# JakubValtar/basisu_rs

Measured on AMD Instinct MI355X. Metric: M 4x4 blocks/s UASTC->BC7 4096x4096, higher is better.
Workload: dtype u8

## Files before the change

### basisu_rs_amd/csrc/bu_capi_slice.hpp

```cpp
#pragma once
extern "C" {

size_t bu_target_block_bytes(bu_target target)
{
    switch (target) {
    case BU_TARGET_ASTC:
    case BU_TARGET_BC7:
    case BU_TARGET_ETC2:
    case BU_TARGET_BC5_RG:
    case BU_TARGET_EAC_RG11:
    case BU_TARGET_BC3_RGBA: return 16;
    case BU_TARGET_ETC1:
    case BU_TARGET_BC4_R:
    case BU_TARGET_EAC_R11:
    case BU_TARGET_BC1_RGB: return 8;
    case BU_TARGET_RGBA32: return 64;
    default: return 0;
    }
}

const char* bu_status_string(bu_status st)
{
    switch (st) {
    case BU_OK: return "ok";
// ... 132 lines not shown
    if (st != BU_ERR_INVALID_MODE && st != BU_ERR_INVALID_PATTERN && st != BU_ERR_INDEX_RANGE && st != BU_ERR_UNSUPPORTED) return BU_ERR_ARGUMENT;
    if (first_bad_block) *first_bad_block = word >> 8;
    return static_cast<bu_status>(st);
}

bu_status bu_host_alloc(bu_context* ctx, size_t bytes, void** out_ptr)
{
    if (!ctx || !out_ptr) return BU_ERR_ARGUMENT;
    *out_ptr = nullptr;
    if (bytes == 0) return BU_OK;
    BU_HIP(ctx, hipSetDevice(ctx->device));
    BU_HIP(ctx, hipHostMalloc(out_ptr, bytes, hipHostMallocDefault));
    return BU_OK;
}

bu_status bu_host_free(bu_context* ctx, void* ptr)
{
    if (!ctx) return BU_ERR_ARGUMENT;
    if (!ptr) return BU_OK;
    BU_HIP(ctx, hipSetDevice(ctx->device));
    BU_HIP(ctx, hipHostFree(ptr));
    return BU_OK;
}

bu_status bu_uastc_transcode_device(bu_context* ctx, bu_target target, const void* d_in, size_t n_blocks, void* d_out,
                                    size_t blocks_per_row, uint64_t block_index_base, uint64_t* d_status, void* stream)
{
    if (!ctx || (n_blocks && (!d_in || !d_out))) return BU_ERR_ARGUMENT;
    if (bu_target_block_bytes(target) == 0) return BU_ERR_ARGUMENT;
    if (target == BU_TARGET_RGBA32 && blocks_per_row == 0) return BU_ERR_ARGUMENT;
    if (target == BU_TARGET_RGBA32 && n_blocks % blocks_per_row != 0) return BU_ERR_ARGUMENT;
    return bu_launch_uastc(ctx, target, d_in, n_blocks, d_out, blocks_per_row, block_index_base, d_status, static_cast<hipStream_t>(stream), 0, -1);
}

}
namespace {
bu_status bu_batch_runs(bu_context* ctx, bu_target target, size_t n_slices, const void* const* d_in, const size_t* n_blocks, void* const* d_out,
                        size_t blocks_per_row, const uint64_t* index_base, std::vector<BuRun>& runs)
{
    if (!ctx || (n_slices && (!d_in || !n_blocks || !d_out))) return BU_ERR_ARGUMENT;
    const size_t bb = bu_target_block_bytes(target);
    if (bb == 0 || (target == BU_TARGET_RGBA32 && blocks_per_row == 0)) return BU_ERR_ARGUMENT;
    for (size_t i = 0; i < n_slices; i++) {
        if (n_blocks[i] && (!d_in[i] || !d_out[i])) return BU_ERR_ARGUMENT;
        if (target == BU_TARGET_RGBA32 && n_blocks[i] % blocks_per_row != 0) return BU_ERR_ARGUMENT;
    }
    bu_merge_runs(n_slices, d_in, n_blocks, d_out, bb, index_base, runs);
    return BU_OK;
}

bu_status bu_launch_runs(bu_context* ctx, bu_target target, const BuRun* runs, size_t n_runs, size_t blocks_per_row, uint64_t* d_status, hipStream_t s, int policy)
{
    if (n_runs == 0) return BU_OK;
    if (n_runs == 1) return bu_launch_uastc(ctx, target, runs[0].in, runs[0].n, runs[0].out, blocks_per_row, runs[0].base, d_status, s, 0, policy);
    if (bu_target_block_bytes(target) == 0) return BU_ERR_ARGUMENT;
    BU_HIP(ctx, hipSetDevice(ctx->device));
    unsigned long long* stw = reinterpret_cast<unsigned long long*>(d_status);
    const unsigned cu_count = (unsigned)ctx->cu_count;
    const size_t bb = bu_target_block_bytes(target);
    std::vector<BuRunsLaunch> plan;
    bu_plan_runs(target, runs, n_runs, blocks_per_row, cu_count, plan);
    for (BuRunsLaunch& l : plan) {
        if (l.plain_run != SIZE_MAX) {
            const BuRun& r = runs[l.plain_run];
            const bu_status st = bu_launch_uastc(ctx, target, r.in, r.n, r.out, blocks_per_row, r.base, d_status, s, 0, policy);
            if (st) return st;
            continue;
        }
        int pol = policy < 0 ? ctx->launch_policy.load(std::memory_order_relaxed) : policy;
        if (pol == BU_POLICY_AUTO) pol = l.needs_policy ? bu_auto_policy(ctx, s) : (int)BU_POLICY_EXCLUSIVE;
        bu_plan_multi_kernel(target, pol, cu_count, l);
        BuRunTable tb;
        for (size_t i = 0; i < l.k; i++) {
            const BuRunEntry& e = l.entries[i];
            const BuRun& r = runs[e.run];
            tb.run[i] = BuRunDesc{reinterpret_cast<const uint4*>(r.in + e.offset * 16), r.out + e.offset * bb, r.base + e.offset, (uint32_t)e.n, e.vshift};
            tb.first_tile[i] = e.first_tile;
        }
        for (size_t i = l.k; i < BU_MULTI_RUNS + 32; i++) tb.first_tile[i] = 0xFFFFFFFFu;
        for (size_t i = l.k; i < BU_MULTI_RUNS; i++) tb.run[i] = BuRunDesc{nullptr, nullptr, 0, 0u, BU_RUN_STRIPS};
        const BuMultiFn k = bu_multi_kernels[target][l.kernel];
        if (!k) return BU_ERR_ARGUMENT;
        unsigned* const ticket = l.wants_ticket ? bu_ticket_for(ctx, s) : nullptr;
        hipLaunchKernelGGL(k, dim3(l.grid), dim3(l.block), 0, s, tb, (unsigned)l.n_tiles, (unsigned)blocks_per_row, stw, ctx->d_tables, ticket);
        const hipError_t e = hipGetLastError();
        if (e != hipSuccess) return bu_fail(ctx, e, "multi-run launch");
    }
    return BU_OK;
}
}
extern "C" {

bu_status bu_uastc_transcode_batch_device(bu_context* ctx, bu_target target, size_t n_slices, const void* const* d_in,
                                          const size_t* n_blocks, void* const* d_out, size_t blocks_per_row,
                                          const uint64_t* index_base, uint64_t* d_status, void* stream)
{
    std::vector<BuRun> runs;
    const bu_status st = bu_batch_runs(ctx, target, n_slices, d_in, n_blocks, d_out, blocks_per_row, index_base, runs);
    if (st) return st;
    return bu_launch_runs(ctx, target, runs.data(), runs.size(), blocks_per_row, d_status, static_cast<hipStream_t>(stream), -1);
}

bu_status bu_uastc_transcode_rects_device(bu_context* ctx, bu_target target, size_t n_jobs, const bu_rect_job* jobs, uint64_t* d_status, void* stream)
{
    if (!ctx || bu_target_block_bytes(target) == 0 || (n_jobs && !jobs)) return BU_ERR_ARGUMENT;
    if (n_jobs == 0) return BU_OK;
    std::vector<BuRectJobIn> in(n_jobs);
    for (size_t i = 0; i < n_jobs; i++) {
        const bu_rect_job& j = jobs[i];
        in[i] = BuRectJobIn{reinterpret_cast<uint64_t>(j.d_in), j.in_blocks_per_row, j.x0, j.y0, j.w, j.h, reinterpret_cast<uint64_t>(j.d_out), j.out_pitch_bytes, j.index_base};
        if (!bu_rect_job_ok(target, in[i])) return BU_ERR_ARGUMENT;
    }
    const BuRectsFn k = bu_rects_kernels[target];
    if (!k) return BU_ERR_ARGUMENT;
    hipStream_t s = static_cast<hipStream_t>(stream);
    BU_HIP(ctx, hipSetDevice(ctx->device));
    const unsigned cu_count = (unsigned)ctx->cu_count;
    std::vector<BuRectsLaunch> plan;
    bu_plan_rects(target, in.data(), n_jobs, plan);
    for (BuRectsLaunch& l : plan) {
        int pol = ctx->launch_policy.load(std::memory_order_relaxed);
        const bool big = bu_rects_needs_policy(l, cu_count);
        if (pol == BU_POLICY_AUTO) pol = big ? bu_auto_policy(ctx, s) : (int)BU_POLICY_EXCLUSIVE;
        else if (big) bu_note_big_enqueue(ctx, s);
        bu_plan_rects_grid(target, pol, cu_count, l);
        hipLaunchKernelGGL(k, dim3(l.grid), dim3(l.block), 0, s, l.table, (unsigned)l.n_tiles, reinterpret_cast<unsigned long long*>(d_status), ctx->d_tables);
        const hipError_t e = hipGetLastError();
        if (e != hipSuccess) return bu_fail(ctx, e, "rectangle launch");
    }
    return BU_OK;
}

}
namespace {
bu_status bu_enqueue_groups(bu_context* ctx, bu_target target, const std::vector<BuRun>& runs, const std::vector<BuRun>& extra, const std::vector<BuLaunchGroup>& groups,
                            size_t first, size_t step, size_t blocks_per_row, uint64_t* d_status, hipStream_t s, int policy)
{
    for (size_t j = first; j < groups.size(); j += step) {
        const BuLaunchGroup& g = groups[j];
        const BuRun* r = g.first >= runs.size() ? &extra[g.first - runs.size()] : &runs[g.first];
        const bu_status st = bu_launch_runs(ctx, target, r, g.count, blocks_per_row, d_status, s, policy);
        if (st) return st;
    }
    return BU_OK;
}

constexpr size_t BU_ENQUEUE_THREADS_MIN_LAUNCHES = 256;

bu_status bu_issue_in_flight(bu_context* ctx, bu_target target, const std::vector<BuRun>& runs, const std::vector<BuRun>& extra, const std::vector<BuLaunchGroup>& groups,
                             size_t blocks_per_row, uint64_t* d_status, int n_streams, int policy)
{
    hipStream_t ss[8];
    for (int i = 0; i < n_streams; i++) ss[i] = ctx->extra_streams[i].load(std::memory_order_acquire);
    if (n_streams > 1 && groups.size() >= BU_ENQUEUE_THREADS_MIN_LAUNCHES && !ctx->single_thread_enqueue.load(std::memory_order_relaxed)) {
        bu_status sts[8] = {BU_OK, BU_OK, BU_OK, BU_OK, BU_OK, BU_OK, BU_OK, BU_OK};
        std::vector<std::thread> th;
        int started = 1;
        for (int si = 1; si < n_streams; si++) {
            try {
                th.emplace_back([&, si] {
                    if (hipSetDevice(ctx->device) != hipSuccess) {
                        sts[si] = bu_fail(ctx, hipGetLastError(), "hipSetDevice");
                        return;
                    }
                    sts[si] = bu_enqueue_groups(ctx, target, runs, extra, groups, (size_t)si, (size_t)n_streams, blocks_per_row, d_status, ss[si], policy);
                });
                started++;
// ... 409 lines not shown
```

### basisu_rs_amd/csrc/bu_kernels.hpp

```cpp
#pragma once
namespace {

constexpr unsigned bu_lds_front(int target) { return target == 1 ? (unsigned)sizeof(BuBc7Tables) : 0u; }
constexpr unsigned bu_lds_table_bytes(int target) { return bu_lds_front(target) + bu_table_bytes(target); }
template <int WGS, int TARGET>
__device__ __forceinline__ void bu_stage_tables_n(uint4* dst, const BuTablesAll* __restrict__ src)
{
    constexpr BuTableRange R = bu_table_range(TARGET);
    constexpr int F = (int)bu_lds_front(TARGET) / 16;
    const uint4* s = reinterpret_cast<const uint4*>(TARGET == 1 ? reinterpret_cast<const void*>(src) : reinterpret_cast<const void*>(&src->t));
    uint4* d = dst;
    for (int i = threadIdx.x; i < F + (int)(R.hi / 16); i += WGS)
        if (i < F || i >= F + (int)(R.lo / 16)) d[i] = s[i];
    if constexpr (R.lo2 < R.hi2) {
        for (int i = F + R.lo2 / 16 + threadIdx.x; i < F + (int)(R.hi2 / 16); i += WGS) d[i] = s[i];
    }
}

__device__ __forceinline__ void bu_report(unsigned long long* status, unsigned long long block, int st)
{
    if (status) (void)__hip_atomic_fetch_min(status, (block << 8) | (unsigned long long)st, __ATOMIC_RELAXED, __HIP_MEMORY_SCOPE_SYSTEM);
}

typedef unsigned int bu_v4u __attribute__((ext_vector_type(4)));
// ... 56 lines not shown
    bu_v4u r;
    r.x = v.x; r.y = v.y; r.z = v.z; r.w = v.w;
#if BU_ST_MODE == 0
    __builtin_nontemporal_store(r, (bu_global_out_v4u)((bu_global_out_bytes)base + off));
#elif BU_ST_MODE == 1
    *(bu_global_out_v4u)((bu_global_out_bytes)base + off) = r;
#else
    asm volatile("global_store_dwordx4 %0, %1, %2" BU_ST_BITS "\n\ts_nop 1" ::"v"(off), "v"(r), "s"(base) : "memory");
#endif
}
__device__ __forceinline__ void bu_st_stream(uint64_t base, uint32_t off, const uint2 v)
{
    bu_v2u r;
    r.x = v.x; r.y = v.y;
#if BU_ST_MODE == 1
    *(bu_global_out_v2u)((bu_global_out_bytes)base + off) = r;
#else
    __builtin_nontemporal_store(r, (bu_global_out_v2u)((bu_global_out_bytes)base + off));
#endif
}

template <int TARGET>
__global__ __launch_bounds__(BU_WG) void bu_uastc_kernel(const uint4* __restrict__ in, void* __restrict__ out, size_t n_blocks,
                                                         unsigned bpr, unsigned long long base, unsigned long long* status,
                                                         const BuTablesAll* __restrict__ tables)
{
    __shared__ uint4 t_store[bu_lds_table_bytes(TARGET) / 16];
    BuTables& T = *reinterpret_cast<BuTables*>(t_store + bu_lds_front(TARGET) / 16);
    const size_t stride = (size_t)gridDim.x * BU_WG;
    size_t idx = (size_t)blockIdx.x * BU_WG + threadIdx.x;
    uint4 v = idx < n_blocks ? bu_ld_stream(in + idx) : make_uint4(0, 0, 0, 0);
    bu_stage_tables_n<BU_WG, TARGET>(t_store, tables);
    __syncthreads();
    while (idx < n_blocks) {
        const size_t next = idx + stride;
        const uint4 vn = next < n_blocks ? in[next] : make_uint4(0, 0, 0, 0);
        BuBlk b;
        b.w[0] = v.x;
        b.w[1] = v.y;
        b.w[2] = v.z;
        b.w[3] = v.w;
        const uint32_t mode = T.mode_lut[v.x & 127u];
        uint32_t o[TARGET == BU_TGT_RGBA ? 16 : 4];
#pragma unroll
        for (int i = 0; i < (TARGET == BU_TGT_RGBA ? 16 : 4); i++) o[i] = 0;
        const int st = bu_block_any<TARGET>(T, mode, b, o);
        if (st) {
            bu_report(status, base + idx, st);
#pragma unroll
            for (int i = 0; i < (TARGET == BU_TGT_RGBA ? 16 : 4); i++) o[i] = 0;
        }
        if constexpr (bu_out_words(TARGET) == 2) {
            reinterpret_cast<uint2*>(out)[idx] = make_uint2(o[0], o[1]);
        } else if constexpr (TARGET == BU_TGT_RGBA) {
            const size_t by = idx / bpr, bx = idx - by * bpr;
            uint4* img = reinterpret_cast<uint4*>(out);
#pragma unroll
            for (int r = 0; r < 4; r++) img[(4 * by + r) * (size_t)bpr + bx] = make_uint4(o[4 * r], o[4 * r + 1], o[4 * r + 2], o[4 * r + 3]);
        } else {
            reinterpret_cast<uint4*>(out)[idx] = make_uint4(o[0], o[1], o[2], o[3]);
        }
        v = vn;
        idx = next;
    }
}

__device__ __forceinline__ uint32_t bu_scan32(uint32_t v)
{
    v += (uint32_t)__builtin_amdgcn_update_dpp(0, (int)v, 0x111, 0xf, 0xf, false);
    v += (uint32_t)__builtin_amdgcn_update_dpp(0, (int)v, 0x112, 0xf, 0xf, false);
    v += (uint32_t)__builtin_amdgcn_update_dpp(0, (int)v, 0x114, 0xf, 0xf, false);
    v += (uint32_t)__builtin_amdgcn_update_dpp(0, (int)v, 0x118, 0xf, 0xf, false);
    v += (uint32_t)__builtin_amdgcn_update_dpp(0, (int)v, 0x142, 0xa, 0xf, false);
    return v;
}

struct BuRunDesc {
    const uint4* in;
    void* out;
    uint64_t base;
    uint32_t n;
    uint32_t vshift;
};
struct BuRunTable {
    BuRunDesc run[BU_MULTI_RUNS];
    uint32_t first_tile[BU_MULTI_RUNS + 32];
};
static_assert(sizeof(BuRunDesc) == 32 && sizeof(BuRunTable) <= 3968, "the run table must fit the 4 KiB of kernel arguments beside the other parameters");
struct BuNoTile {};
template <class TILE>
struct BuWalk {
    TILE d = {}, l = {};
};
template <int BPT>
struct BuMultiWalk : BuWalk<BuMultiTile> {
    uint32_t off[BPT] = {};
    uint32_t off_width = 0xFFFFFFFFu;
    BuRunCursor cur = bu_no_run();
};
enum { BU_LAYOUT_STRIP = 0, BU_LAYOUT_RECT = 1, BU_LAYOUT_MULTI = 2,
       BU_LAYOUT_MULTI_WHOLE = 3,
       BU_LAYOUT_RECTS = 4 };
constexpr unsigned BU_TICKET_STRIDE = 32, BU_TICKET_DONE = 8 * BU_TICKET_STRIDE, BU_TICKET_WORDS = 9 * BU_TICKET_STRIDE;
template <int TARGET, int WGS, int BPT, bool PREFETCH, int LAYOUT>
__device__ __forceinline__ void bu_uastc_sorted_body(const uint4* __restrict__ in, void* __restrict__ out, unsigned n_blocks,
                                                     unsigned bpr, unsigned long long base, unsigned long long* status,
                                                     const BuTablesAll* __restrict__ tables, unsigned cus, unsigned tile_rt,
                                                     const BuRunTable* __restrict__ runs, unsigned* __restrict__ ticket = nullptr,
                                                     const BuRectTable* __restrict__ rects = nullptr)
{
    if (cus != 0) {
        constexpr bool ROT = TARGET == BU_TGT_BC7 || TARGET == BU_TGT_ASTC;
        if (blockIdx.x >= 3 * cus) __builtin_amdgcn_s_setprio(ROT ? 1 : 3);
        else if (blockIdx.x >= 2 * cus) __builtin_amdgcn_s_setprio(2);
        else if (blockIdx.x >= cus) __builtin_amdgcn_s_setprio(ROT ? 3 : 1);
    }
    constexpr int BU_WG = WGS, BU_BPT = BPT, BU_TILE = WGS * BPT;
    __shared__ uint4 t_store[bu_lds_table_bytes(TARGET) / 16];
    BuTables& T = *reinterpret_cast<BuTables*>(t_store + bu_lds_front(TARGET) / 16);
    constexpr bool RECT = LAYOUT == BU_LAYOUT_RECT, MULTI = LAYOUT == BU_LAYOUT_MULTI || LAYOUT == BU_LAYOUT_MULTI_WHOLE;
    constexpr bool WHOLE = RECT || LAYOUT == BU_LAYOUT_MULTI_WHOLE;
    constexpr bool RECTS = LAYOUT == BU_LAYOUT_RECTS;
    static_assert(!RECTS || (BU_TILE == (int)BU_RECTS_TILE && PREFETCH), "the host numbers 1024-block tiles of rectangles; one compiled shape");
    constexpr uint32_t RECTS_ROW_BYTES = bu_rect_row_bytes(TARGET), RECTS_ROWS = bu_rect_rows_per_block(TARGET);
    constexpr bool BU_ALIAS = TARGET == BU_TGT_RGBA;
    static_assert(!BU_ALIAS || bu_lds_table_bytes(TARGET) + 4 * BU_TILE * 16 + BU_TILE + 1536 <= 80 * 1024,
                  "the RGBA32 workgroup no longer fits twice per CU: shrink BuTables or stage it per target in LDS too");
    __shared__ uint4 sblk_store[BU_ALIAS ? 1 : BU_TILE];
    __shared__ uint4 sout[BU_ALIAS ? 4 * BU_TILE : 1];
    uint4* const sblk = BU_ALIAS ? sout : sblk_store;
    constexpr bool INBLOCK = TARGET == BU_TGT_BC7 || TARGET == BU_TGT_ASTC;
    __shared__ uint8_t sst[INBLOCK ? 16 : BU_TILE];
    __shared__ uint32_t cnt[2][32], next_chunk[2];
    const unsigned tid = threadIdx.x, lane = tid & 63u;
    constexpr bool DYN_TILE = bu_dyn_tile(TARGET, BU_TILE) && LAYOUT != BU_LAYOUT_RECT;
    const unsigned tile_blocks = DYN_TILE ? tile_rt : (unsigned)BU_TILE;
    const unsigned n_tiles = (n_blocks + tile_blocks - 1) / tile_blocks;
    auto in_tile = [&](unsigned l) { return !DYN_TILE || l < tile_blocks; };
    static_assert(!RECT || BU_TILE % BU_RECT_W == 0, "rectangular tiles are BU_RECT_W blocks wide and of fixed size");
    const unsigned tpr = RECT ? bpr / BU_RECT_W : 1u;
    auto tile_xy = [&](unsigned t, unsigned& ty, unsigned& tx) {
        ty = (unsigned)(((unsigned long long)t * tile_rt) >> 32);
        tx = t - ty * tpr;
    };
    auto gidx = [&](unsigned t, unsigned l) {
        if constexpr (RECT) {
            unsigned ty, tx;
            tile_xy(t, ty, tx);
            return ((unsigned)(BU_TILE / BU_RECT_W) * ty + l / BU_RECT_W) * bpr + BU_RECT_W * tx + (l % BU_RECT_W);
        } else {
            return t * tile_blocks + l;
        }
    };
    auto has_block = [&](uint32_t k) { return WHOLE || k < 20u; };
    unsigned tile = blockIdx.x;
    __shared__ uint32_t s_next_tile[2];
    uint32_t my_draw = 0;
    unsigned* const my_counter = ticket ? ticket + (blockIdx.x & 7u) * BU_TICKET_STRIDE : nullptr;
    auto tile_of_draw = [&](uint32_t d) { return gridDim.x + 8u * d + (blockIdx.x & 7u); };
    if (ticket && tid == 0) my_draw = atomicAdd(my_counter, 1u);
    using Tile = std::conditional_t<MULTI, BuMultiTile, std::conditional_t<RECTS, BuRectTile, BuNoTile>>;
    std::conditional_t<MULTI, BuMultiWalk<BPT>, BuWalk<Tile>> w;
    constexpr uint32_t OUT_BYTES = TARGET == BU_TGT_RGBA ? 16u : (uint32_t)bu_out_words(TARGET) * 4u;
    constexpr bool RUNS_IN_LDS = (MULTI || RECTS) && PREFETCH;
    __shared__ uint4 s_runs[RUNS_IN_LDS ? (RECTS ? sizeof(BuRectTable) : sizeof(BuRunTable)) / 16 : 1];
    const BuRunTable* R = runs;
    const BuRectTable* Q = rects;
    if constexpr (RUNS_IN_LDS && RECTS) {
        for (unsigned i = tid; i < sizeof(BuRectTable) / 16; i += WGS) s_runs[i] = reinterpret_cast<const uint4*>(rects)[i];
    } else if constexpr (RUNS_IN_LDS) {
        static_assert(sizeof(BuRunTable) % 16 == 0, "copied in 16-byte pieces");
        for (unsigned i = tid; i < sizeof(BuRunTable) / 16; i += WGS) s_runs[i] = reinterpret_cast<const uint4*>(runs)[i];
    }
    auto uni32 = [](uint32_t x) { return (uint32_t)__builtin_amdgcn_readfirstlane((int)x); };
    auto uni64 = [&](uint64_t x) { return (uint64_t)uni32((uint32_t)x) | ((uint64_t)uni32((uint32_t)(x >> 32)) << 32); };
    auto look_up = [&](unsigned t) {
        if constexpr (MULTI) {
            if (t < n_tiles) {
                if (!bu_cursor_holds(w.cur, t)) {
                    uint32_t r = 0;
                    uint32_t ln = lane;
                    asm volatile("" : "+v"(ln));
#pragma unroll
                    for (unsigned c = 0; c < BU_MULTI_RUNS + 32; c += 64) {
                        const uint32_t cnt = (uint32_t)__popcll(__ballot(R->first_tile[c + ln] <= t));
                        if (cnt) r = c + cnt - 1u;
                    }
                    r = (uint32_t)__builtin_amdgcn_readfirstlane((int)r);
                    const BuRunDesc rv = R->run[r];
                    const BuRunRec rd = {uni64(reinterpret_cast<uint64_t>(rv.in)), uni64(reinterpret_cast<uint64_t>(rv.out)), uni64(rv.base), uni32(rv.n), uni32(rv.vshift)};
                    w.cur = bu_run_cursor(rd, uni32(R->first_tile[r]), (uint32_t)BU_TILE);
                }
                w.l = bu_tile_of(w.cur, t, (uint32_t)BU_TILE, OUT_BYTES, TARGET == BU_TGT_RGBA ? bpr : 0u);
                if (w.l.width != w.off_width) {
                    w.off_width = w.l.width;
#pragma unroll
                    for (int j = 0; j < BPT; j++) w.off[j] = bu_lane_off(WHOLE, w.l.width, (unsigned)(j * WGS) + tid);
                }
            }
        } else if constexpr (RECTS) {
            if (t < n_tiles) {
                static_assert(BU_RECT_JOBS == 64, "one first-tile number per lane");
                const uint32_t r = uni32((uint32_t)__popcll(__ballot(Q->first_tile[lane] <= t)) - 1u);
                const BuRectDesc jv = Q->job[r];
                const BuRectDesc jd = {uni64(jv.in), uni64(jv.out), uni64(jv.pitch), uni64(jv.base), uni32(jv.in_bpr), uni32(jv.w), uni32(jv.h), uni32(jv.tpr)};
                w.l = bu_rect_tile(jd, t - uni32(Q->first_tile[r]), RECTS_ROW_BYTES, RECTS_ROWS);
            }
        }
    };
    auto advance = [&] { w.d = w.l; };
    look_up(tile);
    advance();
    auto has_blk = [&](const Tile& d, unsigned t, unsigned l) {
        if constexpr (WHOLE) return true;
        else if constexpr (RECTS) return bu_rect_has(d, l);
        else if constexpr (MULTI) return l < d.n;
        else return t * tile_blocks + l < n_blocks && in_tile(l);
    };
    auto ld_blk = [&](unsigned t, int j) {
        if constexpr (MULTI) return bu_ld_stream_global(w.l.in, w.off[j]);
        else if constexpr (RECTS) return bu_ld_stream_global(reinterpret_cast<const uint4*>(bu_rect_src(w.l, (unsigned)(j * WGS) + tid)));
        else return bu_ld_stream(in + gidx(t, (unsigned)(j * WGS) + tid));
    };
    auto ld_or_zero = [&](unsigned t, int j) { return ((t < n_tiles) & has_blk(w.l, t, (unsigned)(j * WGS) + tid)) ? ld_blk(t, j) : make_uint4(0, 0, 0, 0); };
    constexpr BuTableRange TR = bu_table_range(TARGET);
    constexpr bool SPLIT = bu_lds_table_bytes(TARGET) > 16384;
    constexpr int TF = (int)bu_lds_front(TARGET) / 16, TV1 = (int)(TR.hi - TR.lo) / 16, TV2 = TR.lo2 < TR.hi2 ? (int)(TR.hi2 - TR.lo2) / 16 : 0;
    constexpr int TVT = TF + TV1 + TV2, TVN = (TVT + WGS - 1) / WGS;
    const uint4* const tsrc = reinterpret_cast<const uint4*>(TARGET == BU_TGT_BC7 ? reinterpret_cast<const void*>(tables) : reinterpret_cast<const void*>(&tables->t));
    auto tdst = [&](int i) { return i < TF ? i : (i < TF + TV1 ? (int)(TR.lo / 16) + i : TF + (int)(TR.lo2 / 16) + (i - TF - TV1)); };
    uint4 tv[TVN];
    if constexpr (!SPLIT) {
#pragma unroll
        for (int k = 0; k < TVN; k++) {
            const int i = k * WGS + (int)tid;
            tv[k] = i < TVT ? tsrc[tdst(i)] : make_uint4(0, 0, 0, 0);
        }
    }
    uint4 v[BU_BPT];
#pragma unroll
    for (int j = 0; j < BU_BPT; j++) v[j] = RECT ? ld_blk(tile, j) : ld_or_zero(tile, j);
    if constexpr (!SPLIT) {
#pragma unroll
        for (int k = 0; k < TVN; k++) {
            const int i = k * WGS + (int)tid;
            if (i < TVT) t_store[tdst(i)] = tv[k];
        }
    } else {
#pragma unroll
        for (int k = 0; k < TVN; k++) {
            const int i = k * WGS + (int)tid;
            tv[k] = i < TVT ? tsrc[tdst(i)] : make_uint4(0, 0, 0, 0);
        }
        static_assert(offsetof(BuTables, key_lut) % 4 == 0 && sizeof(T.key_lut[0]) == 128, "the target's key_lut is staged as 32 dwords");
        if (tid < 32) reinterpret_cast<uint32_t*>(T.key_lut[bu_cost_row(TARGET)])[tid] = reinterpret_cast<const uint32_t*>(tables->t.key_lut[bu_cost_row(TARGET)])[tid];
    }
    bool tables_staged = !SPLIT;
    if (tid < 64) (&cnt[0][0])[tid] = 0;
    if (tid < 2) next_chunk[tid] = 0;
    __syncthreads();
    if constexpr (RUNS_IN_LDS && RECTS) Q = reinterpret_cast<const BuRectTable*>(s_runs);
    else if constexpr (RUNS_IN_LDS) R = reinterpret_cast<const BuRunTable*>(s_runs);
    unsigned par = 0;
    unsigned next_of_loop = 0;
    constexpr bool STORES_LAST = PREFETCH && MULTI && (TARGET == BU_TGT_BC7 || (TARGET == BU_TGT_ASTC && WGS == 256 && WHOLE));
    auto key_of = [&](const Tile& d, unsigned t, int j, uint32_t x) { return has_blk(d, t, (unsigned)(j * BU_WG) + tid) ? (uint32_t)T.key_lut[bu_cost_row(TARGET)][x & 127u] : 31u; };
    uint32_t next_key[STORES_LAST ? BU_BPT : 1];
    uint32_t drawn_tile = 0;
    if constexpr (STORES_LAST) {
        if (tile < n_tiles) {
#pragma unroll
            for (int j = 0; j < BU_BPT; j++) next_key[j] = key_of(w.d, tile, j, v[j].x);
        }
        if (ticket && tid == 0) drawn_tile = tile_of_draw(my_draw);
        __builtin_amdgcn_s_waitcnt(0x0F70);
    }
    for (; tile < n_tiles; tile = next_of_loop, par ^= 1u) {
        uint32_t key[BU_BPT], pos[BU_BPT];
        bool uniform = true;
#pragma unroll
        for (int j = 0; j < BU_BPT; j++) {
            key[j] = STORES_LAST ? next_key[j] : key_of(w.d, tile, j, v[j].x);
            uniform = uniform && (__ballot(key[j] == (uint32_t)__builtin_amdgcn_readfirstlane(key[j])) == ~0ull) && has_block(key[j]);
        }
        if (uniform) {
            uint32_t lead[BU_BPT];
#pragma unroll
            for (int j = 0; j < BU_BPT; j++) lead[j] = lane == 0 ? atomicAdd(&cnt[par][key[j]], 64u) : 0u;
#pragma unroll
            for (int j = 0; j < BU_BPT; j++) pos[j] = (uint32_t)__builtin_amdgcn_readfirstlane(lead[j]) + lane;
        } else {
#pragma unroll
            for (int j = 0; j < BU_BPT; j++) pos[j] = atomicAdd(&cnt[par][key[j]], 1u);
        }
        if (ticket && tid == 0) s_next_tile[par] = STORES_LAST ? drawn_tile : tile_of_draw(my_draw);
        if (!tables_staged) {
#pragma unroll
            for (int k = 0; k < TVN; k++) {
                const int i = k * WGS + (int)tid;
                if (i < TVT) t_store[tdst(i)] = tv[k];
            }
            tables_staged = true;
        }
        __syncthreads();
        const uint32_t run_c = lane < 20u ? cnt[par][lane] : 0u;
        const uint32_t run_pk = run_c | (((run_c + 63u) >> 6) << 16);
        const uint32_t run_incl = bu_scan32(run_pk), run_excl = run_incl - run_pk;
        const uint32_t nc = (uint32_t)__builtin_amdgcn_readlane((int)run_incl, 31) >> 16;
        if (tid < 32) cnt[par ^ 1u][tid] = 0;
        if (tid == 0) next_chunk[par ^ 1u] = 0;
        uint32_t dest[BU_BPT];
#pragma unroll
        for (int j = 0; j < BU_BPT; j++) {
            const uint32_t st = (uint32_t)__builtin_amdgcn_ds_bpermute((int)(key[j] << 2), (int)run_excl) & 0xFFFFu;
            dest[j] = has_block(key[j]) ? st + pos[j] : 0u;
            if (has_block(key[j])) sblk[dest[j]] = v[j];
        }
        const unsigned ntile = ticket ? (unsigned)__builtin_amdgcn_readfirstlane((int)s_next_tile[par]) : tile + gridDim.x;
        next_of_loop = ntile;
        uint4 vn[BU_BPT];
        if constexpr (PREFETCH) {
            look_up(ntile);
            if constexpr (MULTI && WHOLE) {
                if (ntile < n_tiles) {
#pragma unroll
                    for (int j = 0; j < BU_BPT; j++) vn[j] = ld_blk(ntile, j);
                } else {
#pragma unroll
                    for (int j = 0; j < BU_BPT; j++) vn[j] = make_uint4(0, 0, 0, 0);
                }
            } else {
#pragma unroll
                for (int j = 0; j < BU_BPT; j++) vn[j] = ld_or_zero(ntile, j);
            }
        }
        if (ticket && tid == 0 && ntile < n_tiles) my_draw = atomicAdd(my_counter, 1u);
        __syncthreads();
        uint32_t c_next = 0;
        if (lane == 0) c_next = atomicAdd(&next_chunk[par], 1u);
        for (;;) {
            const uint32_t c = __builtin_amdgcn_readfirstlane(c_next);
            if (c >= nc) break;
            if (lane == 0) c_next = atomicAdd(&next_chunk[par], 1u);
            const uint32_t r = (uint32_t)__builtin_ctzll(__ballot((run_incl >> 16) > c));
            const uint32_t r_pk = (uint32_t)__builtin_amdgcn_readlane((int)run_pk, (int)r), r_ex = (uint32_t)__builtin_amdgcn_readlane((int)run_excl, (int)r);
            const uint32_t k64 = (c - (r_ex >> 16)) << 6;
            const uint32_t s0 = (r_ex & 0xFFFFu) + k64, left = (r_pk & 0xFFFFu) - k64, count = left < 64u ? left : 64u;
            const bool active = lane < count;
            const uint32_t slot = s0 + (active ? lane : 0u);
            const uint4 bv = sblk[slot];
            BuBlk b;
            b.w[0] = bv.x;
            b.w[1] = bv.y;
            b.w[2] = bv.z;
            b.w[3] = bv.w;
            constexpr int NO = TARGET == BU_TGT_RGBA ? 16 : 4;
            uint32_t o[NO];
#pragma unroll
            for (int i = 0; i < NO; i++) o[i] = 0;
            int st = BU_ST_BAD_MODE;
            if (active) {
                switch (r) {
#define BU_CASE(k) \
    case k: st = bu_block_mode<TARGET, BU_COST_ORDER[bu_cost_row(TARGET)][k]>(T, b, o); break;
                    BU_CASE(0) BU_CASE(1) BU_CASE(2) BU_CASE(3) BU_CASE(4) BU_CASE(5) BU_CASE(6) BU_CASE(7) BU_CASE(8) BU_CASE(9)
                    BU_CASE(10) BU_CASE(11) BU_CASE(12) BU_CASE(13) BU_CASE(14) BU_CASE(15) BU_CASE(16) BU_CASE(17) BU_CASE(18)
#undef BU_CASE
                default: break;
                }
                if constexpr (TARGET == BU_TGT_RGBA) {
#pragma unroll
                    for (int r2 = 0; r2 < 4; r2++) sout[r2 * BU_TILE + slot] = make_uint4(o[4 * r2], o[4 * r2 + 1], o[4 * r2 + 2], o[4 * r2 + 3]);
                    sst[slot] = (uint8_t)st;
                } else if constexpr (INBLOCK) {
                    sblk[slot] = make_uint4(o[0], o[1], o[2], o[3] | (uint32_t)st);
                } else {
                    sblk[slot] = make_uint4(o[0], o[1], o[2], o[3]);
                    sst[slot] = (uint8_t)st;
                }
            }
        }
        __syncthreads();
        [[maybe_unused]] uint32_t so[MULTI ? BU_BPT : 1];
        if constexpr (MULTI) {
#pragma unroll
            for (int j = 0; j < BPT; j++) so[j] = w.off[j];
            if (w.d.width != w.off_width) {
#pragma unroll
                for (int j = 0; j < BPT; j++) so[j] = bu_lane_off(WHOLE, w.d.width, (unsigned)(j * WGS) + tid);
            }
        }
        auto blk_of = [&](int j) -> unsigned long long {
            if constexpr (RECTS) return w.d.base + bu_rect_idx(w.d, (unsigned)(j * BU_WG) + tid);
            else if constexpr (MULTI) return w.d.base + bu_lane_block(w.d, so[j]);
            else return base + gidx(tile, (unsigned)(j * BU_WG) + tid);
        };
        auto put16 = [&](int j, const uint4 r) {
            if constexpr (RECTS) bu_st_stream(reinterpret_cast<uint4*>(bu_rect_dst(w.d, (unsigned)(j * BU_WG) + tid, RECTS_ROW_BYTES, RECTS_ROWS)), r);
            else if constexpr (MULTI) bu_st_stream(w.d.out, so[j], r);
            else bu_st_stream(reinterpret_cast<uint4*>(out) + gidx(tile, (unsigned)(j * BU_WG) + tid), r);
        };
        auto put8 = [&](int j, const uint2 r) {
            if constexpr (RECTS) bu_st_stream(reinterpret_cast<uint2*>(bu_rect_dst(w.d, (unsigned)(j * BU_WG) + tid, RECTS_ROW_BYTES, RECTS_ROWS)), r);
            else if constexpr (MULTI) bu_st_stream(w.d.out, so[j] >> 1, r);
            else bu_st_stream(reinterpret_cast<uint2*>(out) + gidx(tile, (unsigned)(j * BU_WG) + tid), r);
        };
        auto put_row = [&](int j, int r, const uint4 px) {
            const unsigned l = (unsigned)(j * BU_WG) + tid;
            if constexpr (RECTS) {
                bu_st_stream(reinterpret_cast<uint4*>(bu_rect_dst(w.d, l, RECTS_ROW_BYTES, RECTS_ROWS) + (uint64_t)r * w.d.pitch), px);
            } else if constexpr (MULTI) {
                bu_st_stream(w.d.out, bu_lane_off_rgba(w.d, so[j], bpr) + (uint32_t)r * bpr * 16u, px);
            } else {
                unsigned by, bx;
                if constexpr (RECT) {
                    unsigned ty, tx;
                    tile_xy(tile, ty, tx);
                    by = (unsigned)(BU_TILE / BU_RECT_W) * ty + l / BU_RECT_W;
                    bx = BU_RECT_W * tx + (l % BU_RECT_W);
                } else {
                    by = gidx(tile, l) / bpr;
                    bx = gidx(tile, l) - by * bpr;
                }
                bu_st_stream(reinterpret_cast<uint4*>(out) + (size_t)((4 * by + r) * bpr + bx), px);
            }
        };
        auto take_inblock = [&](int j) {
            uint4 r = sblk[dest[j]];
            if ((r.x & 0xFFu) == 0u) {
                bu_report(status, blk_of(j), (int)r.w);
                r.w = 0;
            }
            return r;
        };
        if constexpr (STORES_LAST) {
            uint4 r[BU_BPT];
            bool has[BU_BPT];
#pragma unroll
            for (int j = 0; j < BU_BPT; j++) {
                has[j] = has_block(key[j]);
                if (has[j]) r[j] = take_inblock(j);
            }
#pragma unroll
            for (int j = 0; j < BU_BPT; j++) next_key[j] = key_of(w.l, ntile, j, vn[j].x);
            drawn_tile = tile_of_draw(my_draw);
            asm volatile("" : "+v"(drawn_tile));
#pragma unroll
            for (int j = 0; j < BU_BPT; j++)
                if (has[j]) put16(j, r[j]);
        } else {
#pragma unroll
            for (int j = 0; j < BU_BPT; j++) {
                if (!has_block(key[j])) continue;
                if constexpr (INBLOCK) {
                    put16(j, take_inblock(j));
                } else {
                    const uint32_t st = sst[dest[j]];
                    if (st) bu_report(status, blk_of(j), (int)st);
                    if constexpr (TARGET == BU_TGT_RGBA) {
#pragma unroll
                        for (int r = 0; r < 4; r++) put_row(j, r, sout[r * BU_TILE + dest[j]]);
                    } else {
                        const uint4 r = sblk[dest[j]];
                        if constexpr (bu_out_words(TARGET) == 2) put8(j, make_uint2(r.x, r.y));
                        else put16(j, r);
                    }
                }
            }
        }
        if constexpr (PREFETCH) {
#pragma unroll
            for (int j = 0; j < BU_BPT; j++) v[j] = vn[j];
        } else {
            look_up(ntile);
#pragma unroll
            for (int j = 0; j < BU_BPT; j++) v[j] = ld_or_zero(ntile, j);
        }
        advance();
    }
    if (ticket && tid == 0) {
        if (atomicAdd(ticket + BU_TICKET_DONE, 1u) == gridDim.x - 1u) {
            for (unsigned k = 0; k < 8; k++) atomicExch(ticket + k * BU_TICKET_STRIDE, 0u);
            atomicExch(ticket + BU_TICKET_DONE, 0u);
        }
    }
}

template <int TARGET, int WGS, int BPT, int MINW, bool PREFETCH, int LAYOUT>
__global__ __launch_bounds__(WGS, MINW) void bu_uastc_sorted_kernel(const uint4* __restrict__ in, void* __restrict__ out, unsigned n_blocks,
                                                                unsigned bpr, unsigned long long base, unsigned long long* status,
                                                                const BuTablesAll* __restrict__ tables, unsigned cus, unsigned tile_rt,
                                                                unsigned* __restrict__ ticket)
{
    static_assert(LAYOUT != BU_LAYOUT_MULTI && LAYOUT != BU_LAYOUT_MULTI_WHOLE, "several runs per launch: bu_uastc_multi_kernel");
    bu_uastc_sorted_body<TARGET, WGS, BPT, PREFETCH, LAYOUT>(in, out, n_blocks, bpr, base, status, tables, cus, tile_rt, nullptr, ticket);
}

constexpr bool bu_multi_etc_2048(int target, int tile) { return bu_etc_family(target) && tile == 2048; }
template <int TARGET, int WGS, int BPT, bool PREFETCH = false, bool WHOLE = false>
__global__ __launch_bounds__(WGS, (TARGET == BU_TGT_ASTC && WGS == 512) ? 8 : bu_multi_etc_2048(TARGET, WGS * BPT) ? 4 : 1) void bu_uastc_multi_kernel(
    const BuRunTable table, unsigned n_tiles, unsigned bpr, unsigned long long* status, const BuTablesAll* __restrict__ tables, unsigned* __restrict__ ticket)
{
    static_assert(WGS * BPT == 1024 || bu_multi_etc_2048(TARGET, WGS * BPT), "the host numbers 1024-block tiles (ETC1 / ETC2 large batches: 2048-block ones)");
    static_assert(sizeof(BuRunTable) + 40 <= 4096, "the run table and the other arguments share the 4 KiB of kernel arguments");
    bu_uastc_sorted_body<TARGET, WGS, BPT, PREFETCH, WHOLE ? BU_LAYOUT_MULTI_WHOLE : BU_LAYOUT_MULTI>(nullptr, nullptr, n_tiles * (unsigned)(WGS * BPT), bpr, 0ull, status, tables, 0u,
                                                                                                        (unsigned)(WGS * BPT), &table, ticket);
}

template <int TARGET>
__global__ __launch_bounds__(512) void bu_uastc_rects_kernel(const BuRectTable table, unsigned n_tiles, unsigned long long* status, const BuTablesAll* __restrict__ tables)
{
    static_assert(sizeof(BuRectTable) + 24 <= 4096, "the job table and the other arguments share the 4 KiB of kernel arguments");
    bu_uastc_sorted_body<TARGET, 512, 2, true, BU_LAYOUT_RECTS>(nullptr, nullptr, n_tiles * BU_RECTS_TILE, 0u, 0ull, status, tables, 0u, BU_RECTS_TILE, nullptr, nullptr, &table);
}

__global__ void bu_status_reset_kernel(unsigned long long* words, unsigned n)
{
    for (unsigned i = threadIdx.x; i < n; i += blockDim.x) words[i] = ~0ull;
}

struct BuCrcTables {
    uint16_t t[4][256];
    uint16_t pw[256];
};
constexpr unsigned BU_CRC_PIECE = 65536;

__device__ __forceinline__ uint32_t bu_crc_gf_mul(uint32_t a, uint32_t b)
{
    uint32_t r = 0;
#pragma unroll
    for (int i = 15; i >= 0; i--) {
        r <<= 1;
        r ^= (r & 0x10000u) ? 0x11021u : 0u;
        r ^= ((b >> i) & 1u) ? a : 0u;
    }
    return r & 0xFFFFu;
}

__global__ __launch_bounds__(256) void bu_crc16_pieces_kernel(const uint4* __restrict__ data, uint16_t* __restrict__ partial,
                                                              const BuCrcTables* __restrict__ tables)
{
    __shared__ BuCrcTables C;
    __shared__ uint32_t red[4];
    static_assert(sizeof(BuCrcTables) % 16 == 0, "copied in 16-byte pieces");
    for (unsigned i = threadIdx.x; i < sizeof(BuCrcTables) / 16; i += 256) reinterpret_cast<uint4*>(&C)[i] = reinterpret_cast<const uint4*>(tables)[i];
    __syncthreads();
    const uint4* p = data + (size_t)blockIdx.x * (BU_CRC_PIECE / 16) + threadIdx.x * 16;
    uint32_t s = 0;
#pragma unroll 4
    for (int i = 0; i < 16; i++) {
        const uint4 v = p[i];
        const uint32_t w[4] = {v.x, v.y, v.z, v.w};
#pragma unroll
        for (int k = 0; k < 4; k++) {
            const uint32_t x = w[k];
            s = (uint32_t)C.t[3][((s >> 8) ^ x) & 255u] ^ (uint32_t)C.t[2][(s ^ (x >> 8)) & 255u] ^ (uint32_t)C.t[1][(x >> 16) & 255u] ^ (uint32_t)C.t[0][x >> 24];
        }
    }
    uint32_t c = bu_crc_gf_mul(s, C.pw[255u - threadIdx.x]);
#pragma unroll
    for (int d = 32; d >= 1; d >>= 1) c ^= (uint32_t)__shfl_xor((int)c, d);
    if ((threadIdx.x & 63u) == 0) red[threadIdx.x >> 6] = c;
    __syncthreads();
    if (threadIdx.x == 0) partial[blockIdx.x] = (uint16_t)(red[0] ^ red[1] ^ red[2] ^ red[3]);
}

__global__ __launch_bounds__(64) void bu_sleep_kernel(unsigned long long ticks)
{
    const unsigned long long t0 = wall_clock64();
    while (wall_clock64() - t0 < ticks) __builtin_amdgcn_s_sleep(32);
}

template <int WG, int EPT>
__global__ __launch_bounds__(WG) void bu_copy_kernel(const uint4* __restrict__ in, uint4* __restrict__ out, size_t n)
{
    const size_t base = (size_t)blockIdx.x * (WG * EPT) + threadIdx.x;
    uint4 v[EPT];
#pragma unroll
    for (int k = 0; k < EPT; k++) {
        const size_t i = base + (size_t)k * WG;
        if (i < n) v[k] = bu_ld_stream(in + i);
    }
#pragma unroll
    for (int k = 0; k < EPT; k++) {
        const size_t i = base + (size_t)k * WG;
        if (i < n) {
            bu_v4u r;
            r.x = v[k].x; r.y = v[k].y; r.z = v[k].z; r.w = v[k].w;
            __builtin_nontemporal_store(r, reinterpret_cast<bu_v4u*>(out + i));
        }
    }
}

}
```

### basisu_rs_amd/csrc/bu_multi_addr.hpp

```cpp
#pragma once
#include <stdint.h>

#include "bu_launch_plan.hpp"

struct BuRunRec {
    uint64_t in, out, base;
    uint32_t n;
    uint32_t vshift;
};
struct BuRunCursor {
    BuRunRec run;
    uint32_t first_tile, n_tiles;
};
struct BuMultiTile {
    uint64_t in;
    uint64_t out;
    uint64_t base;
    uint32_t first;
    uint32_t n;
    uint32_t width;
    uint32_t bx0;
};

BU_DEV BuRunCursor bu_no_run() { return BuRunCursor{BuRunRec{0, 0, 0, 0u, BU_RUN_STRIPS}, 0u, 0u}; }
BU_DEV BuRunCursor bu_run_cursor(const BuRunRec& r, uint32_t first_tile, uint32_t tile) { return BuRunCursor{r, first_tile, r.n / tile + (r.n % tile ? 1u : 0u)}; }
BU_DEV bool bu_cursor_holds(const BuRunCursor& c, uint32_t t) { return t - c.first_tile < c.n_tiles; }

BU_DEV BuMultiTile bu_tile_of(const BuRunCursor& c, uint32_t t, uint32_t tile, uint32_t out_bytes, uint32_t rgba_bpr)
{
    const BuRunRec& r = c.run;
    const uint32_t lt = t - c.first_tile;
    BuMultiTile d;
    if (r.vshift != BU_RUN_STRIPS) {
        const uint32_t ty = lt >> r.vshift, tx = lt & ((1u << r.vshift) - 1u);
        d.width = (uint32_t)BU_RECT_W << r.vshift;
        d.first = (tile / (uint32_t)BU_RECT_W) * ty * d.width + (uint32_t)BU_RECT_W * tx;
        d.n = tile;
    } else {
        d.width = 0u;
        d.first = lt * tile;
        d.n = r.n - d.first < tile ? r.n - d.first : tile;
    }
    d.in = r.in + (uint64_t)d.first * 16u;
    d.base = r.base;
    if (rgba_bpr) {
        const uint32_t by0 = d.first / rgba_bpr;
        d.bx0 = d.first - by0 * rgba_bpr;
        d.out = r.out + (uint64_t)by0 * rgba_bpr * 64u;
    } else {
        d.bx0 = 0u;
        d.out = r.out + (uint64_t)d.first * out_bytes;
    }
    return d;
}

BU_DEV uint32_t bu_lane_off(bool whole, uint32_t width, uint32_t l)
{
    return ((whole || width) ? (l / (uint32_t)BU_RECT_W) * width + (l % (uint32_t)BU_RECT_W) : l) * 16u;
}
static_assert((uint64_t)((2048 / BU_RECT_W - 1) * (uint64_t)BU_MULTI_MAX_WIDTH + BU_RECT_W - 1) * 16u < ((uint64_t)1 << 32), "a lane offset fits 32 bits");
BU_DEV uint64_t bu_lane_block(const BuMultiTile& d, uint32_t off) { return (uint64_t)d.first + (off >> 4); }

BU_DEV uint32_t bu_lane_off_rgba(const BuMultiTile& d, uint32_t off, uint32_t bpr)
{
    const uint32_t c = d.bx0 + (off >> 4), dy = c / bpr;
    return (3u * dy * bpr + c) * 16u;
}
static_assert((7 * (uint64_t)BU_MULTI_RGBA_MAX_BPR + 4 * ((2048 / BU_RECT_W) * (uint64_t)BU_MULTI_MAX_WIDTH)) * 16u < ((uint64_t)1 << 32), "an RGBA32 lane offset fits 32 bits");

inline uint32_t bu_run_of_tile(const uint32_t* first_tile, uint32_t entries, uint32_t t)
{
    uint32_t cnt = 0;
    for (uint32_t i = 0; i < entries; i++) cnt += first_tile[i] <= t;
    return cnt - 1u;
}
```

Baseline: 192,300.

## Resolve first run in kernel prologue from scalar head args and overlap LDS staging

Passes the first 14 entries of the run table's first_tile array as separate scalar kernel arguments, so each workgroup can find its first run with scalar compares instead of an initial lookup. The per-tile placement logic is split out so the first tile is placed directly from that precomputed run. The run-table copy into LDS is now loaded into registers before the barrier and overlapped with the table staging, and the ticket atomic is moved later. gridDim is replaced by an explicit grid_size held in scalar registers. This shortens the kernel prologue at the cost of more kernel arguments and register pressure.

New measurement: 193,000 (median of 6 runs). About the same (+0.4%).

```diff
diff --git a/basisu_rs_amd/csrc/bu_capi_slice.hpp b/basisu_rs_amd/csrc/bu_capi_slice.hpp
--- a/basisu_rs_amd/csrc/bu_capi_slice.hpp
+++ b/basisu_rs_amd/csrc/bu_capi_slice.hpp
@@ -238,7 +238,10 @@
         const BuMultiFn k = bu_multi_kernels[target][l.kernel];
         if (!k) return BU_ERR_ARGUMENT;
         unsigned* const ticket = l.wants_ticket ? bu_ticket_for(ctx, s) : nullptr;
-        hipLaunchKernelGGL(k, dim3(l.grid), dim3(l.block), 0, s, tb, (unsigned)l.n_tiles, (unsigned)blocks_per_row, stw, ctx->d_tables, ticket);
+        static_assert(BU_RUN_HEAD == 14, "one leading argument per entry of the head");
+        const uint32_t* const h = tb.first_tile;
+        hipLaunchKernelGGL(k, dim3(l.grid), dim3(l.block), 0, s, h[0], h[1], h[2], h[3], h[4], h[5], h[6], h[7], h[8], h[9], h[10], h[11], h[12], h[13], tb,
+                           (unsigned)l.n_tiles, (unsigned)blocks_per_row, stw, ctx->d_tables, ticket);
         const hipError_t e = hipGetLastError();
         if (e != hipSuccess) return bu_fail(ctx, e, "multi-run launch");
     }
diff --git a/basisu_rs_amd/csrc/bu_kernels.hpp b/basisu_rs_amd/csrc/bu_kernels.hpp
--- a/basisu_rs_amd/csrc/bu_kernels.hpp
+++ b/basisu_rs_amd/csrc/bu_kernels.hpp
@@ -162,7 +162,7 @@
     uint32_t n;
     uint32_t vshift;
 };
-struct BuRunTable {
+struct alignas(16) BuRunTable {
     BuRunDesc run[BU_MULTI_RUNS];
     uint32_t first_tile[BU_MULTI_RUNS + 32];
 };
@@ -185,9 +185,9 @@
 template <int TARGET, int WGS, int BPT, bool PREFETCH, int LAYOUT>
 __device__ __forceinline__ void bu_uastc_sorted_body(const uint4* __restrict__ in, void* __restrict__ out, unsigned n_blocks,
                                                      unsigned bpr, unsigned long long base, unsigned long long* status,
-                                                     const BuTablesAll* __restrict__ tables, unsigned cus, unsigned tile_rt,
+                                                     const BuTablesAll* __restrict__ tables, unsigned cus, unsigned tile_rt, uint32_t grid_size,
                                                      const BuRunTable* __restrict__ runs, unsigned* __restrict__ ticket = nullptr,
-                                                     const BuRectTable* __restrict__ rects = nullptr)
+                                                     const BuRectTable* __restrict__ rects = nullptr, const BuRunRec first_run = {}, uint32_t first_run_tile = 0)
 {
     if (cus != 0) {
         constexpr bool ROT = TARGET == BU_TGT_BC7 || TARGET == BU_TGT_ASTC;
@@ -237,23 +237,32 @@
     __shared__ uint32_t s_next_tile[2];
     uint32_t my_draw = 0;
     unsigned* const my_counter = ticket ? ticket + (blockIdx.x & 7u) * BU_TICKET_STRIDE : nullptr;
-    auto tile_of_draw = [&](uint32_t d) { return gridDim.x + 8u * d + (blockIdx.x & 7u); };
-    if (ticket && tid == 0) my_draw = atomicAdd(my_counter, 1u);
+    auto tile_of_draw = [&](uint32_t d) { return grid_size + 8u * d + (blockIdx.x & 7u); };
     using Tile = std::conditional_t<MULTI, BuMultiTile, std::conditional_t<RECTS, BuRectTile, BuNoTile>>;
     std::conditional_t<MULTI, BuMultiWalk<BPT>, BuWalk<Tile>> w;
     constexpr uint32_t OUT_BYTES = TARGET == BU_TGT_RGBA ? 16u : (uint32_t)bu_out_words(TARGET) * 4u;
     constexpr bool RUNS_IN_LDS = (MULTI || RECTS) && PREFETCH;
-    __shared__ uint4 s_runs[RUNS_IN_LDS ? (RECTS ? sizeof(BuRectTable) : sizeof(BuRunTable)) / 16 : 1];
+    constexpr int RUNS_PIECES = RUNS_IN_LDS ? (int)(RECTS ? sizeof(BuRectTable) : sizeof(BuRunTable)) / 16 : 0, RVN = (RUNS_PIECES + WGS - 1) / WGS;
+    static_assert(sizeof(BuRunTable) % 16 == 0 && sizeof(BuRectTable) % 16 == 0, "copied in 16-byte pieces");
+    __shared__ uint4 s_runs[RUNS_IN_LDS ? RUNS_PIECES : 1];
     const BuRunTable* R = runs;
     const BuRectTable* Q = rects;
-    if constexpr (RUNS_IN_LDS && RECTS) {
-        for (unsigned i = tid; i < sizeof(BuRectTable) / 16; i += WGS) s_runs[i] = reinterpret_cast<const uint4*>(rects)[i];
-    } else if constexpr (RUNS_IN_LDS) {
-        static_assert(sizeof(BuRunTable) % 16 == 0, "copied in 16-byte pieces");
-        for (unsigned i = tid; i < sizeof(BuRunTable) / 16; i += WGS) s_runs[i] = reinterpret_cast<const uint4*>(runs)[i];
-    }
     auto uni32 = [](uint32_t x) { return (uint32_t)__builtin_amdgcn_readfirstlane((int)x); };
     auto uni64 = [&](uint64_t x) { return (uint64_t)uni32((uint32_t)x) | ((uint64_t)uni32((uint32_t)(x >> 32)) << 32); };
+    auto place = [&](unsigned t) {
+        if constexpr (MULTI) {
+            w.l = bu_tile_of(w.cur, t, (uint32_t)BU_TILE, OUT_BYTES, TARGET == BU_TGT_RGBA ? bpr : 0u);
+            if constexpr (TARGET == BU_TGT_RGBA) {
+                w.l.out = uni64(w.l.out);
+                w.l.bx0 = uni32(w.l.bx0);
+            }
+            if (w.l.width != w.off_width) {
+                w.off_width = w.l.width;
+#pragma unroll
+                for (int j = 0; j < BPT; j++) w.off[j] = bu_lane_off(WHOLE, w.l.width, (unsigned)(j * WGS) + tid);
+            }
+        }
+    };
     auto look_up = [&](unsigned t) {
         if constexpr (MULTI) {
             if (t < n_tiles) {
@@ -271,12 +280,7 @@
                     const BuRunRec rd = {uni64(reinterpret_cast<uint64_t>(rv.in)), uni64(reinterpret_cast<uint64_t>(rv.out)), uni64(rv.base), uni32(rv.n), uni32(rv.vshift)};
                     w.cur = bu_run_cursor(rd, uni32(R->first_tile[r]), (uint32_t)BU_TILE);
                 }
-                w.l = bu_tile_of(w.cur, t, (uint32_t)BU_TILE, OUT_BYTES, TARGET == BU_TGT_RGBA ? bpr : 0u);
-                if (w.l.width != w.off_width) {
-                    w.off_width = w.l.width;
-#pragma unroll
-                    for (int j = 0; j < BPT; j++) w.off[j] = bu_lane_off(WHOLE, w.l.width, (unsigned)(j * WGS) + tid);
-                }
+                place(t);
             }
         } else if constexpr (RECTS) {
             if (t < n_tiles) {
@@ -289,7 +293,12 @@
         }
     };
     auto advance = [&] { w.d = w.l; };
-    look_up(tile);
+    if constexpr (MULTI) {
+        w.cur = bu_run_cursor(first_run, first_run_tile, (uint32_t)BU_TILE);
+        if (tile < n_tiles) place(tile);
+    } else {
+        look_up(tile);
+    }
     advance();
     auto has_blk = [&](const Tile& d, unsigned t, unsigned l) {
         if constexpr (WHOLE) return true;
@@ -320,6 +329,25 @@
     uint4 v[BU_BPT];
 #pragma unroll
     for (int j = 0; j < BU_BPT; j++) v[j] = RECT ? ld_blk(tile, j) : ld_or_zero(tile, j);
+    [[maybe_unused]] uint32_t key_lut_v = 0;
+    if constexpr (SPLIT) {
+#pragma unroll
+        for (int k = 0; k < TVN; k++) {
+            const int i = k * WGS + (int)tid;
+            tv[k] = i < TVT ? tsrc[tdst(i)] : make_uint4(0, 0, 0, 0);
+        }
+        static_assert(offsetof(BuTables, key_lut) % 4 == 0 && sizeof(T.key_lut[0]) == 128, "the target's key_lut is staged as 32 dwords");
+        if (tid < 32) key_lut_v = reinterpret_cast<const uint32_t*>(tables->t.key_lut[bu_cost_row(TARGET)])[tid];
+    }
+    [[maybe_unused]] uint4 runs_v[RVN ? RVN : 1];
+    if constexpr (RUNS_IN_LDS) {
+        const uint4* const rsrc = RECTS ? reinterpret_cast<const uint4*>(rects) : reinterpret_cast<const uint4*>(runs);
+#pragma unroll
+        for (int k = 0; k < RVN; k++) {
+            const int i = k * WGS + (int)tid;
+            runs_v[k] = i < RUNS_PIECES ? rsrc[i] : make_uint4(0, 0, 0, 0);
+        }
+    }
     if constexpr (!SPLIT) {
 #pragma unroll
         for (int k = 0; k < TVN; k++) {
@@ -327,17 +355,20 @@
             if (i < TVT) t_store[tdst(i)] = tv[k];
         }
     } else {
-#pragma unroll
-        for (int k = 0; k < TVN; k++) {
+        if (tid < 32) reinterpret_cast<uint32_t*>(T.key_lut[bu_cost_row(TARGET)])[tid] = key_lut_v;
+    }
+    if constexpr (RUNS_IN_LDS) {
+#pragma unroll
+        for (int k = 0; k < RVN; k++) {
             const int i = k * WGS + (int)tid;
-            tv[k] = i < TVT ? tsrc[tdst(i)] : make_uint4(0, 0, 0, 0);
-        }
-        static_assert(offsetof(BuTables, key_lut) % 4 == 0 && sizeof(T.key_lut[0]) == 128, "the target's key_lut is staged as 32 dwords");
-        if (tid < 32) reinterpret_cast<uint32_t*>(T.key_lut[bu_cost_row(TARGET)])[tid] = reinterpret_cast<const uint32_t*>(tables->t.key_lut[bu_cost_row(TARGET)])[tid];
+            if (i < RUNS_PIECES) s_runs[i] = runs_v[k];
+        }
     }
     bool tables_staged = !SPLIT;
     if (tid < 64) (&cnt[0][0])[tid] = 0;
     if (tid < 2) next_chunk[tid] = 0;
+    if (ticket && tid == 0) my_draw = atomicAdd(my_counter, 1u);
+    if constexpr (!MULTI) asm volatile("" : "+s"(grid_size));
     __syncthreads();
     if constexpr (RUNS_IN_LDS && RECTS) Q = reinterpret_cast<const BuRectTable*>(s_runs);
     else if constexpr (RUNS_IN_LDS) R = reinterpret_cast<const BuRunTable*>(s_runs);
@@ -396,7 +427,7 @@
             dest[j] = has_block(key[j]) ? st + pos[j] : 0u;
             if (has_block(key[j])) sblk[dest[j]] = v[j];
         }
-        const unsigned ntile = ticket ? (unsigned)__builtin_amdgcn_readfirstlane((int)s_next_tile[par]) : tile + gridDim.x;
+        const unsigned ntile = ticket ? (unsigned)__builtin_amdgcn_readfirstlane((int)s_next_tile[par]) : tile + grid_size;
         next_of_loop = ntile;
         uint4 vn[BU_BPT];
         if constexpr (PREFETCH) {
@@ -559,7 +590,7 @@
         advance();
     }
     if (ticket && tid == 0) {
-        if (atomicAdd(ticket + BU_TICKET_DONE, 1u) == gridDim.x - 1u) {
+        if (atomicAdd(ticket + BU_TICKET_DONE, 1u) == grid_size - 1u) {
             for (unsigned k = 0; k < 8; k++) atomicExch(ticket + k * BU_TICKET_STRIDE, 0u);
             atomicExch(ticket + BU_TICKET_DONE, 0u);
         }
@@ -573,25 +604,36 @@
                                                                 unsigned* __restrict__ ticket)
 {
     static_assert(LAYOUT != BU_LAYOUT_MULTI && LAYOUT != BU_LAYOUT_MULTI_WHOLE, "several runs per launch: bu_uastc_multi_kernel");
-    bu_uastc_sorted_body<TARGET, WGS, BPT, PREFETCH, LAYOUT>(in, out, n_blocks, bpr, base, status, tables, cus, tile_rt, nullptr, ticket);
+    bu_uastc_sorted_body<TARGET, WGS, BPT, PREFETCH, LAYOUT>(in, out, n_blocks, bpr, base, status, tables, cus, tile_rt, gridDim.x, nullptr, ticket);
 }
 
 constexpr bool bu_multi_etc_2048(int target, int tile) { return bu_etc_family(target) && tile == 2048; }
 template <int TARGET, int WGS, int BPT, bool PREFETCH = false, bool WHOLE = false>
 __global__ __launch_bounds__(WGS, (TARGET == BU_TGT_ASTC && WGS == 512) ? 8 : bu_multi_etc_2048(TARGET, WGS * BPT) ? 4 : 1) void bu_uastc_multi_kernel(
-    const BuRunTable table, unsigned n_tiles, unsigned bpr, unsigned long long* status, const BuTablesAll* __restrict__ tables, unsigned* __restrict__ ticket)
+    unsigned h0, unsigned h1, unsigned h2, unsigned h3, unsigned h4, unsigned h5, unsigned h6, unsigned h7, unsigned h8, unsigned h9, unsigned h10, unsigned h11,
+    unsigned h12, unsigned h13, const BuRunTable table, unsigned n_tiles, unsigned bpr, unsigned long long* status, const BuTablesAll* __restrict__ tables,
+    unsigned* __restrict__ ticket)
 {
     static_assert(WGS * BPT == 1024 || bu_multi_etc_2048(TARGET, WGS * BPT), "the host numbers 1024-block tiles (ETC1 / ETC2 large batches: 2048-block ones)");
-    static_assert(sizeof(BuRunTable) + 40 <= 4096, "the run table and the other arguments share the 4 KiB of kernel arguments");
+    static_assert(sizeof(BuRunTable) + 64 + 40 <= 4096,"the run table and the other arguments share the 4 KiB of kernel arguments");
+    static_assert(BU_RUN_HEAD == 14, "one leading argument per entry of the head");
+    const uint32_t head[BU_RUN_HEAD] = {h0, h1, h2, h3, h4, h5, h6, h7, h8, h9, h10, h11, h12, h13};
+    const uint32_t r = bu_run_of_tile_scalar(head, table.first_tile, blockIdx.x);
+    const BuRunDesc& rv = table.run[r];
+    const BuRunRec first_run = {reinterpret_cast<uint64_t>(rv.in), reinterpret_cast<uint64_t>(rv.out), rv.base, rv.n, rv.vshift};
+    const uint32_t first_run_tile = table.first_tile[r];
+    uint32_t grid_size = gridDim.x;
+    asm volatile("" : "+s"(n_tiles), "+s"(grid_size) : "s"(first_run.in), "s"(first_run.out), "s"(first_run.base), "s"(first_run.n), "s"(first_run.vshift), "s"(first_run_tile), "s"(bpr),
+                 "s"(tables), "s"(ticket));
     bu_uastc_sorted_body<TARGET, WGS, BPT, PREFETCH, WHOLE ? BU_LAYOUT_MULTI_WHOLE : BU_LAYOUT_MULTI>(nullptr, nullptr, n_tiles * (unsigned)(WGS * BPT), bpr, 0ull, status, tables, 0u,
-                                                                                                        (unsigned)(WGS * BPT), &table, ticket);
+                                                                                                        (unsigned)(WGS * BPT), grid_size, &table, ticket, nullptr, first_run, first_run_tile);
 }
 
 template <int TARGET>
 __global__ __launch_bounds__(512) void bu_uastc_rects_kernel(const BuRectTable table, unsigned n_tiles, unsigned long long* status, const BuTablesAll* __restrict__ tables)
 {
     static_assert(sizeof(BuRectTable) + 24 <= 4096, "the job table and the other arguments share the 4 KiB of kernel arguments");
-    bu_uastc_sorted_body<TARGET, 512, 2, true, BU_LAYOUT_RECTS>(nullptr, nullptr, n_tiles * BU_RECTS_TILE, 0u, 0ull, status, tables, 0u, BU_RECTS_TILE, nullptr, nullptr, &table);
+    bu_uastc_sorted_body<TARGET, 512, 2, true, BU_LAYOUT_RECTS>(nullptr, nullptr, n_tiles * BU_RECTS_TILE, 0u, 0ull, status, tables, 0u, BU_RECTS_TILE, gridDim.x, nullptr, nullptr, &table);
 }
 
 __global__ void bu_status_reset_kernel(unsigned long long* words, unsigned n)
diff --git a/basisu_rs_amd/csrc/bu_multi_addr.hpp b/basisu_rs_amd/csrc/bu_multi_addr.hpp
--- a/basisu_rs_amd/csrc/bu_multi_addr.hpp
+++ b/basisu_rs_amd/csrc/bu_multi_addr.hpp
@@ -74,3 +74,23 @@
     for (uint32_t i = 0; i < entries; i++) cnt += first_tile[i] <= t;
     return cnt - 1u;
 }
+
+constexpr uint32_t BU_RUN_HEAD = 14;
+static_assert(BU_RUN_HEAD + (BU_MULTI_RUNS - BU_RUN_HEAD + 15) / 16 * 16 <= BU_MULTI_RUNS + 32, "the last chunk of the scalar search stays inside first_tile[]");
+BU_DEV uint32_t bu_run_of_tile_scalar(const uint32_t* head, const uint32_t* first_tile, uint32_t t)
+{
+    uint32_t cnt = 0;
+    BU_UNROLL
+    for (uint32_t i = 0; i < BU_RUN_HEAD; i++) cnt += head[i] <= t;
+    if (cnt == BU_RUN_HEAD) {
+#pragma unroll 1
+        for (uint32_t c = BU_RUN_HEAD; c < BU_MULTI_RUNS; c += 16) {
+            uint32_t k = 0;
+            BU_UNROLL
+            for (uint32_t i = 0; i < 16; i++) k += first_tile[c + i] <= t;
+            cnt += k;
+            if (k < 16) break;
+        }
+    }
+    return cnt - 1u;
+}
```
